# in3otd/glfer

Hardware: AMD Instinct MI355X
Metric: spectrogram frames/sec + achieved HBM GB/s, N=4096 MTM K=4 (higher is better)
Workload: dtype f32

## Files before the change

glfer_amd/csrc/odd_taper.hpp:

```cpp
#pragma once
#include "stockham16.hpp"

#ifndef GLFER_PSD_STORE_AUX
#define GLFER_PSD_STORE_AUX 0
#endif

namespace glfer {

template <int FMT, int T, int HIST = -1>
__device__ __forceinline__ void load_frame16(const SpectroParams &p, unsigned t, unsigned fl, long long fblk, float (&dst)[16]) {
  constexpr unsigned esz = FMT == GLFER_FMT_F32 ? 4 : (FMT == GLFER_FMT_S16 ? 2 : 1);
  const long long f = fblk + fl;
  const unsigned flc = f < p.nframes ? fl : (unsigned)(p.nframes - 1 - fblk);
  const long long sblk = (p.frame0 + fblk) * (long long)p.H - p.R;
  if (HIST == 1 || (HIST < 0 && p.history_mode)) {
    const __amdgpu_buffer_rsrc_t hrsrc = __builtin_amdgcn_make_buffer_rsrc(
        const_cast<char *>(reinterpret_cast<const char *>(p.stream)) + (sblk + p.R) * (long long)esz, 0, 0x7fffffff, 0x00020000);
    const int d = (int)t - p.R;
    const int lrel = (int)(flc * (unsigned)p.H) + d;
    static_for<0, 16>([&](auto mc) {
      constexpr int m = decltype(mc)::value;
      const bool ok = d >= -T * m;
      const float x = buf_sample<FMT>(hrsrc, ok ? (unsigned)(lrel + T * m) * esz : 0x80000000u, 0u);
      dst[m] = ok ? x : 0.0f;
    });
    return;
  }
  const __amdgpu_buffer_rsrc_t xrsrc = __builtin_amdgcn_make_buffer_rsrc(
      const_cast<char *>(reinterpret_cast<const char *>(p.stream)) + sblk * (long long)esz, 0, 0x7fffffff, 0x00020000);
  const unsigned lrel = flc * (unsigned)p.H + t;
  static_for<0, 16>([&](auto mc) {
    constexpr int m = decltype(mc)::value;
    dst[m] = buf_sample<FMT>(xrsrc, lrel * esz, (unsigned)(T * m) * esz);
  });
}

__device__ __forceinline__ float wave_total_f32(float v) {
  auto dpp = [](float x, auto ctrl, auto rowmask) {
    return __int_as_float(__builtin_amdgcn_update_dpp(0, __float_as_int(x), decltype(ctrl)::value, decltype(rowmask)::value, 0xf, false));
  };
  v += dpp(v, std::integral_constant<int, 0x111>{}, std::integral_constant<int, 0xf>{});
  v += dpp(v, std::integral_constant<int, 0x112>{}, std::integral_constant<int, 0xf>{});
  v += dpp(v, std::integral_constant<int, 0x114>{}, std::integral_constant<int, 0xf>{});
  v += dpp(v, std::integral_constant<int, 0x118>{}, std::integral_constant<int, 0xf>{});
  v += dpp(v, std::integral_constant<int, 0x142>{}, std::integral_constant<int, 0xa>{});
  v += dpp(v, std::integral_constant<int, 0x143>{}, std::integral_constant<int, 0xc>{});
  return __int_as_float(__builtin_amdgcn_readlane(__float_as_int(v), 63));
}

template <int FMT, int T, int KM>
__device__ __forceinline__ void load_frame16_mean(const SpectroParams &p, unsigned t, unsigned fl, long long fblk, float (&dst)[16]) {
  static_assert(T <= 64 && (KM == 16 || KM == 8 || KM == 4), "a frame within one wavefront; hop = 4, 8 or 16 registers");
  load_frame16<FMT, T, 0>(p, t, fl, fblk, dst);
  constexpr int NH = 16 / KM;
  float mu[NH];
  if (p.means) {
    const long long f = fblk + fl;
    const long long F = p.frame0 + (f < p.nframes ? f : (long long)p.nframes - 1);
#pragma unroll
    for (int q = 0; q < NH; q++) mu[q] = p.means[F - (NH - 1) + q];
  } else {
#pragma unroll
    for (int q = 0; q < NH; q++) {
      float sm = 0.0f;
#pragma unroll
      for (int m = 0; m < KM; m++) sm += dst[q * KM + m];
#pragma unroll
      for (int o = 1; o < T; o <<= 1) sm += __shfl_xor(sm, o);
      mu[q] = sm / (float)p.H;
    }
  }
#pragma unroll
  for (int m = 0; m < 16; m++) dst[m] = dst[m] - mu[m / KM];
}

constexpr int kSilent = 0x7fff;
__device__ __forceinline__ int scale_exponent(float power) {
  int ex = __builtin_amdgcn_frexp_expf(power);
  ex = ex > 120 ? 120 : (ex < -120 ? -120 : ex);
  return power == 0.0f ? kSilent : ex >> 1;
}
__device__ __forceinline__ float scale_in(int hx) { return hx == kSilent ? 0.0f : __builtin_amdgcn_ldexpf(1.0f, -hx); }
__device__ __forceinline__ float scale_out(int hx) { return hx == kSilent ? 0.0f : __builtin_amdgcn_ldexpf(1.0f, 2 * hx); }

template <int LOGN, int FPB, class SumA, class SumB>
__device__ __forceinline__ void separate_and_store(const SpectroParams &p, const float (&zr)[16], const float (&zi)[16],
                                                   v2f32 *xb, unsigned t, unsigned fl, long long fblk, int hxA, int hxB,
                                                   SumA &&sumA, SumB &&sumB) {
  using C = Plan16<LOGN>;
  constexpr int N = C::N, T = C::T, RL = C::radix(C::NPASS - 1), BL = 16 / RL;
  auto rho_of = [](int m) constexpr { return (m % BL) + BL * brev(m / BL, RL); };
  if constexpr (GLFER16_BARRIER_AFTER_READS == 0) frame_sync<T>();
  static_for<8, 16>([&](auto mc) {
    constexpr int m = decltype(mc)::value;
    constexpr int r = rho_of(m);
    xb[t + T * (m - 8)] = v2f32{zr[r], zi[r]};
  });
  frame_sync<T>();
  const unsigned ROWB = (unsigned)p.pitch * 4u;
  const long long leftA = p.nframes - fblk, leftB = p.nframes - (fblk + FPB);
  const unsigned recA = (unsigned)((leftA > FPB ? FPB : leftA) * (long long)ROWB);
  const unsigned recB = leftB > 0 ? (unsigned)((leftB > FPB ? FPB : leftB) * (long long)ROWB) : 0u;
  const __amdgpu_buffer_rsrc_t ra = __builtin_amdgcn_make_buffer_rsrc(p.psd + (size_t)fblk * (size_t)p.pitch, 0, recA, 0x00020000);
  const __amdgpu_buffer_rsrc_t rb = __builtin_amdgcn_make_buffer_rsrc(p.psd + (size_t)(fblk + (leftB > 0 ? FPB : 0)) * (size_t)p.pitch, 0, recB, 0x00020000);
  const unsigned voff = fl * ROWB + t * 4u;
  const float uA = scale_out(hxA), uB = scale_out(hxB);
  static_for<0, 8>([&](auto mc) {
    constexpr int m = decltype(mc)::value;
    constexpr int r = rho_of(m);
    const int k = (int)t + T * m;
    v2f32 b = xb[N / 2 - k];
    const float ar = zr[r], ai = zi[r];
    if constexpr (m == 0) {
      if (t == 0) b = v2f32{ar, ai};
    }
    const float er = ar + b.x, ei = ai - b.y, orr = ar - b.x, oi = ai + b.y;
    const float pa = __builtin_fmaf(er, er, ei * ei), pb = __builtin_fmaf(orr, orr, oi * oi);
    __builtin_amdgcn_raw_buffer_store_b32(__float_as_uint(__builtin_fmaf(pa, uA, sumA(mc))), ra, voff, (unsigned)(T * m) * 4u, GLFER_PSD_STORE_AUX);
    __builtin_amdgcn_raw_buffer_store_b32(__float_as_uint(__builtin_fmaf(pb, uB, sumB(mc))), rb, voff, (unsigned)(T * m) * 4u, GLFER_PSD_STORE_AUX);
  });
  if (t == 0) {
    constexpr int r = rho_of(8);
    constexpr std::integral_constant<int, 8> nyq{};
    __builtin_amdgcn_raw_buffer_store_b32(__float_as_uint(__builtin_fmaf(4.0f * zr[r] * zr[r], uA, sumA(nyq))), ra, voff, (unsigned)(N / 2) * 4u, GLFER_PSD_STORE_AUX);
    __builtin_amdgcn_raw_buffer_store_b32(__float_as_uint(__builtin_fmaf(4.0f * zi[r] * zi[r], uB, sumB(nyq))), rb, voff, (unsigned)(N / 2) * 4u, GLFER_PSD_STORE_AUX);
  }
  frame_sync<T>();
}

}
```

glfer_amd/csrc/spectro16y.hip:

```cpp
#include <hip/hip_runtime.h>
#include <stdint.h>
#include "odd_taper.hpp"

#ifndef GLFER16Y_DPP_SUM
#define GLFER16Y_DPP_SUM 1
#endif
#ifndef GLFER16Y_SKEW
#define GLFER16Y_SKEW 1
#endif
#ifndef GLFER16Y_HALF
#define GLFER16Y_HALF 1
#endif
#ifndef GLFER16Y_TW1_REGS
#define GLFER16Y_TW1_REGS 1
#endif

#ifndef GLFER_BLOCK_MARK
#define GLFER_BLOCK_MARK(k)
#endif

#ifdef GLFER_RAGGED
#define spectro16y_kernel spectro16y_ragged_kernel
#define glfer_launch_spectro16y_n12 glfer_launch_spectro16y_ragged_n12
#endif

namespace glfer {

hipError_t allow_dynamic_lds(const void *kernel, size_t bytes);

struct LaunchY {
  static constexpr int N = 4096, T = 256, PADN = N + N / 16;
  static constexpr int LDS_WORDS = 2 * PADN + 16 * 17 + 4;
};

template <int FMT, int ABL = 0, int HIST = 0, int KM = 0, int BAT = 0, int HALF = 0, int QUEUE = 0>
__global__ __launch_bounds__(256, 2) void spectro16y_kernel(SpectroParams p) {
  GLFER_BLOCK_MARK(0);
  if constexpr (KM == 0 || BAT != 0) GLFER_STREAM_SELECT(p);
  static_assert(KM == 0 || (HIST == 0 && (KM == 16 || KM == 8 || KM == 4)), "in-kernel mean removal: history from the stream");
  static_assert(HALF == 0 || (KM == 0 && GLFER16_X0_ROWS != 0 && GLFER16_BARRIER_AFTER_READS != 0), "half tables: the plain forms, row layout of exchange 0");
  static_assert(QUEUE == 0 || (KM == 0 && BAT == 0 && ABL == 0), "frame queue: the plain single-stream forms");
  constexpr int NH = KM > 0 ? 16 / KM : 1;
  __shared__ float mred[KM > 0 ? 4 * (NH + 1) : 1];
  using C = Plan16<12>;
  using L = LaunchY;
  constexpr int N = L::N, T = L::T, PADN = L::PADN, NPASS = C::NPASS;
  constexpr int TW1 = 15;
  constexpr int NT = C::NTW - TW1;
  constexpr unsigned esz = FMT == GLFER_FMT_F32 ? 4 : (FMT == GLFER_FMT_S16 ? 2 : 1);
  typedef float v4f32 __attribute__((ext_vector_type(4)));
  extern __shared__ v2f32 lds[];

  const unsigned t = threadIdx.x;
  const unsigned rc = HALF ? glfer_yhalf_residue(t) : t;
  v2f32 *xbA = lds, *xbB = lds + PADN;
  v2f32 *tw1 = lds + 2 * PADN;
  float *red = reinterpret_cast<float *>(lds + 2 * PADN + 16 * 17);

  {
    const v2f32 *tw = reinterpret_cast<const v2f32 *>(p.tw);
    const unsigned k = t >> 4, q = t & 15;
    tw1[k * 17 + q] = q ? tw[(q - 1) * T + k] : v2f32{1.0f, 0.0f};
  }
  float twr[NT], twi[NT];
  {
    const v2f32 *tw = reinterpret_cast<const v2f32 *>(p.tw) + t;
#pragma unroll
    for (int e = 0; e < NT; e++) {
      const v2f32 w = tw[(TW1 + e) * T];
      twr[e] = w.x;
      twi[e] = w.y;
    }
  }
  __syncthreads();
  const v2f32 *tw1row = tw1 + (t & 15) * 17;
  constexpr bool TW1R = GLFER16Y_TW1_REGS != 0 && HIST == 0 && KM != 4;
  v2f32 tw1reg[16];
  if constexpr (TW1R) {
#pragma unroll
    for (int q = 0; q < 16; q++) tw1reg[q] = tw1row[q];
  }

  const __amdgpu_buffer_rsrc_t trsrc = __builtin_amdgcn_make_buffer_rsrc(
      const_cast<float *>(p.taps), 0, p.npairs * 2 * N * 4, 0x00020000);
  const __amdgpu_buffer_rsrc_t vrsrc = __builtin_amdgcn_make_buffer_rsrc(
      const_cast<float *>(p.xtaps), 0, N * 4, 0x00020000);
  const unsigned toff = t * 16u;
  const int NP = p.npairs - 1;
  const long long stride = (long long)gridDim.x * 2;

  auto load_x = [&](float (&dst)[16], long long f) {
    load_frame16<FMT, T, HIST>(p, rc, 0u, f < p.nframes ? f : (long long)p.nframes - 1, dst);
  };
  v2f32 pt[16];
  auto prefetch_taps = [&](int pair) {
    const unsigned tap_p = (unsigned)pair * (N * 8u);
    static_for<0, 8>([&](auto mc) {
      constexpr int mh = decltype(mc)::value;
      const v4f32 q = __builtin_bit_cast(v4f32, __builtin_amdgcn_raw_buffer_load_b128(trsrc, toff, tap_p + (unsigned)(T * mh) * 16u, 0));
      pt[2 * mh] = v2f32{q.x, q.y};
      pt[2 * mh + 1] = v2f32{q.z, q.w};
    });
  };
  auto prefetch_last = [&] {
    static_for<0, 4>([&](auto mc) {
      constexpr int mq = decltype(mc)::value;
      const v4f32 q = __builtin_bit_cast(v4f32, __builtin_amdgcn_raw_buffer_load_b128(vrsrc, toff, (unsigned)(T * mq) * 16u, 0));
      pt[2 * mq] = v2f32{q.x, q.y};
      pt[2 * mq + 1] = v2f32{q.z, q.w};
    });
  };

  v2f32 hp[16];
  float hl[8];
  const __amdgpu_buffer_rsrc_t yrsrc = __builtin_amdgcn_make_buffer_rsrc(
      const_cast<float *>(p.ytaps), 0, HALF ? T * GLFER_YHALF_FLOATS * 4 : 0, 0x00020000);
  const unsigned yoff = t * (unsigned)(GLFER_YHALF_FLOATS * 4);
  auto load_half_last = [&] {
    static_for<0, 2>([&](auto cc) {
      constexpr int c = decltype(cc)::value;
      const v4f32 q = __builtin_bit_cast(v4f32, __builtin_amdgcn_raw_buffer_load_b128(yrsrc, yoff, 128u + c * 16u, 0));
      hl[4 * c] = q.x;
      hl[4 * c + 1] = q.y;
      hl[4 * c + 2] = q.z;
      hl[4 * c + 3] = q.w;
    });
  };
  if constexpr (HALF != 0) {
    static_for<0, 8>([&](auto cc) {
      constexpr int c = decltype(cc)::value;
      const v4f32 q = __builtin_bit_cast(v4f32, __builtin_amdgcn_raw_buffer_load_b128(yrsrc, yoff, c * 16u, 0));
      hp[2 * c] = v2f32{q.x, q.y};
      hp[2 * c + 1] = v2f32{q.z, q.w};
    });
// ... 7 lines not shown
    if constexpr (m < 8) return hp[P * 8 + m];
    else return v2f32{mirror(hp[P * 8 + 15 - m].x), -mirror(hp[P * 8 + 15 - m].y)};
  };

  const long long span = QUEUE ? 2LL * p.yq_chunk : 2;
  unsigned *qword = reinterpret_cast<unsigned *>(tw1 + 16);
  long long fA = (long long)xcd_block_index() * span;
  if (fA >= p.nframes) return;
  long long fEnd = fA + span < p.nframes ? fA + span : (long long)p.nframes, next_chunk = 0;
  bool fresh = true;
  float xA[16], xB[16];
  load_x(xA, fA);
  if (fA + 1 < p.nframes) load_x(xB, fA + 1);
  else {
#pragma unroll
    for (int m = 0; m < 16; m++) xB[m] = 0.0f;
  }
  if constexpr (HALF == 0) prefetch_taps(0);

  auto publish_hop_sums = [&] {
    static_for<0, NH + 1>([&](auto qc) {
      constexpr int q = decltype(qc)::value;
      float sm = 0.0f;
      static_for<0, KM>([&](auto mc) {
        constexpr int m = decltype(mc)::value;
        sm += q < NH ? xA[q * KM + m] : xB[(NH - 1) * KM + m];
      });
#pragma unroll
      for (int o = 1; o < 64; o <<= 1) sm += __shfl_xor(sm, o);
      if ((t & 63u) == 0) mred[(t >> 6) * (NH + 1) + q] = sm;
    });
  };
  auto subtract_hop_means = [&] {
    float mu[NH + 1];
#pragma unroll
    for (int q = 0; q <= NH; q++)
      mu[q] = ((mred[q] + mred[(NH + 1) + q]) + (mred[2 * (NH + 1) + q] + mred[3 * (NH + 1) + q])) / (float)p.H;
#pragma unroll
    for (int m = 0; m < 16; m++) {
      xA[m] = xA[m] - mu[m / (KM ? KM : 1)];
      xB[m] = xB[m] - mu[m / (KM ? KM : 1) + 1];
    }
  };
  auto subtract_table_means = [&](long long fa) {
    float mu[NH + 1];
    const long long F = p.frame0 + fa;
#pragma unroll
    for (int q = 0; q < NH; q++) mu[q] = p.means[F - (NH - 1) + q];
    mu[NH] = p.means[fa + 1 < p.nframes ? F + 1 : F];
#pragma unroll
    for (int m = 0; m < 16; m++) {
      xA[m] = xA[m] - mu[m / (KM ? KM : 1)];
      xB[m] = xB[m] - mu[m / (KM ? KM : 1) + 1];
    }
  };
  if constexpr (KM > 0) {
    if (p.means) {
      subtract_table_means(fA);
    } else {
      publish_hop_sums();
      __syncthreads();
      subtract_hop_means();
      __syncthreads();
    }
    if (fA + 1 >= p.nframes) {
#pragma unroll
      for (int m = 0; m < 16; m++) xB[m] = 0.0f;
    }
  }

  constexpr int RL = C::radix(NPASS - 1), BL = 16 / RL;
  auto rho_of = [](int m) constexpr { return (m % BL) + BL * brev(m / BL, RL); };

  GLFER_BLOCK_MARK(1);
  while (true) {
    long long nfA = fA + stride;
    bool has_next = nfA < p.nframes;
    unsigned ticket = 0;
    if constexpr (QUEUE != 0) {
      if (fresh && t == 0) ticket = __hip_atomic_fetch_add(p.yq_counter, 1u, __ATOMIC_RELAXED, __HIP_MEMORY_SCOPE_AGENT);
    }
    float psdA[8], psdB[8], nyqA, nyqB;
    int hxA, hxB;
    {
      float accA[16], accB[16];
#pragma unroll
      for (int r = 0; r < 16; r++) accA[r] = accB[r] = 0.0f;
      if constexpr (HALF != 0) {
        static_for<0, 2>([&](auto pc) {
          constexpr int P = decltype(pc)::value;
          float zrA[16], ziA[16], zrB[16], ziB[16];
          GLFER_STAMP(0);
          static_for<0, 16>([&](auto mc) {
            constexpr int m = decltype(mc)::value;
            const v2f32 w = half_pair(pc, mc);
            zrA[m] = xA[m] * w.x;
            ziA[m] = xA[m] * w.y;
            zrB[m] = xB[m] * w.x;
            ziB[m] = xB[m] * w.y;
          });
          auto dual = [&](const auto &tw1sel) {
            auto hook = [] {};
            if constexpr (GLFER16Y_SKEW != 0) stockham16_passes2s<12, NT>(zrA, ziA, xbA, zrB, ziB, xbB, t, rc, tw1sel, twr, twi, hook);
            else stockham16_passes2<12, NT>(zrA, ziA, xbA, zrB, ziB, xbB, t, rc, tw1sel, twr, twi, hook);
          };
          if constexpr (TW1R) dual(tw1reg);
          else dual(tw1row);
#pragma unroll
          for (int r = 0; r < 16; r++) {
            if constexpr (P == 0) {
              accA[r] = __builtin_fmaf(zrA[r], zrA[r], ziA[r] * ziA[r]);
              accB[r] = __builtin_fmaf(zrB[r], zrB[r], ziB[r] * ziB[r]);
            } else {
              accA[r] = __builtin_fmaf(zrA[r], zrA[r], __builtin_fmaf(ziA[r], ziA[r], accA[r]));
              accB[r] = __builtin_fmaf(zrB[r], zrB[r], __builtin_fmaf(ziB[r], ziB[r], accB[r]));
            }
          }
          GLFER_STAMP(15);
        });
        if constexpr (HALF == 2) load_half_last();
      } else
      for (int pair = 0; pair < NP; pair++) {
        float zrA[16], ziA[16], zrB[16], ziB[16];
        GLFER_STAMP(0);
#pragma unroll
        for (int m = 0; m < 16; m++) {
          zrA[m] = xA[m] * pt[m].x;
          ziA[m] = xA[m] * pt[m].y;
          zrB[m] = xB[m] * pt[m].x;
          ziB[m] = xB[m] * pt[m].y;
        }
        auto dual = [&](const auto &tw1sel) {
          auto hook = [&] {
            if (pair + 1 < NP) prefetch_taps(pair + 1);
            else prefetch_last();
          };
          if constexpr (GLFER16Y_SKEW != 0) stockham16_passes2s<12, NT>(zrA, ziA, xbA, zrB, ziB, xbB, t, tw1sel, twr, twi, hook);
          else stockham16_passes2<12, NT>(zrA, ziA, xbA, zrB, ziB, xbB, t, tw1sel, twr, twi, hook);
        };
        if constexpr (TW1R) dual(tw1reg);
        else dual(tw1row);
        if (pair == 0) {
#pragma unroll
          for (int r = 0; r < 16; r++) {
            accA[r] = __builtin_fmaf(zrA[r], zrA[r], ziA[r] * ziA[r]);
            accB[r] = __builtin_fmaf(zrB[r], zrB[r], ziB[r] * ziB[r]);
          }
        } else {
#pragma unroll
          for (int r = 0; r < 16; r++) {
            accA[r] = __builtin_fmaf(zrA[r], zrA[r], __builtin_fmaf(ziA[r], ziA[r], accA[r]));
            accB[r] = __builtin_fmaf(zrB[r], zrB[r], __builtin_fmaf(ziB[r], ziB[r], accB[r]));
          }
        }
        GLFER_STAMP(15);
      }
      float eA = 0.0f, eB = 0.0f;
#pragma unroll
      for (int r = 0; r < 16; r++) {
        eA += accA[r];
        eB += accB[r];
      }
#if GLFER16Y_DPP_SUM
      eA = wave_total_f32(eA);
      eB = wave_total_f32(eB);
#else
#pragma unroll
      for (int w = 1; w < 64; w <<= 1) {
        eA += __shfl_xor(eA, w);
        eB += __shfl_xor(eB, w);
      }
#endif
      float *foldA = reinterpret_cast<float *>(xbA), *foldB = reinterpret_cast<float *>(xbB);
      static_for<8, 16>([&](auto mc) {
        constexpr int m = decltype(mc)::value;
        foldA[t + T * (m - 8)] = accA[rho_of(m)];
        foldB[t + T * (m - 8)] = accB[rho_of(m)];
      });
      if ((t & 63) == 0) {
        red[t >> 6] = eA;
        red[4 + (t >> 6)] = eB;
      }
      if constexpr (QUEUE != 0) {
        if (fresh && t == 0) *qword = ticket - p.yq_base;
      }
      __syncthreads();
      if constexpr (QUEUE != 0) {
        if (fresh) next_chunk = ((long long)gridDim.x + (long long)(unsigned)__builtin_amdgcn_readfirstlane((int)*qword)) * span;
        nfA = fA + 2 < fEnd ? fA + 2 : next_chunk;
        has_next = nfA < p.nframes;
      }
      eA = (red[0] + red[1]) + (red[2] + red[3]);
      eB = (red[4] + red[5]) + (red[6] + red[7]);
      hxA = scale_exponent(eA);
      hxB = scale_exponent(eB);
      static_for<0, 8>([&](auto mc) {
        constexpr int m = decltype(mc)::value;
        const int k = T * m + (int)t;
        float oa = foldA[N / 2 - k], ob = foldB[N / 2 - k];
        if constexpr (m == 0) {
          if (t == 0) {
            oa = accA[rho_of(0)];
            ob = accB[rho_of(0)];
          }
        }
        psdA[m] = accA[rho_of(m)] + oa;
        psdB[m] = accB[rho_of(m)] + ob;
      });
      nyqA = 2.0f * accA[rho_of(8)];
      nyqB = 2.0f * accB[rho_of(8)];
      __syncthreads();
    }

    if constexpr (ABL == 1) {
      if (has_next) {
        if constexpr (HALF == 0) prefetch_taps(0);
        load_x(xA, nfA);
        load_x(xB, nfA + 1);
      }
      if (t == 0) p.psd[(size_t)fA * (size_t)p.pitch] = psdA[0] + psdB[0] + nyqA + nyqB + (float)(hxA + hxB);
      if (!has_next) break;
      fA = nfA;
      continue;
    }
    float zr[16], zi[16];
    GLFER_STAMP(0);
    {
      const float sA = scale_in(hxA), sB = scale_in(hxB);
      if constexpr (HALF != 0) {
        static_for<0, 16>([&](auto mc) {
          constexpr int m = decltype(mc)::value;
          float v;
          if constexpr (m < 8) v = hl[m];
          else v = mirror(hl[15 - m]);
          zr[m] = (xA[m] * v) * sA;
          zi[m] = (xB[m] * v) * sB;
        });
      } else {
#pragma unroll
        for (int m = 0; m < 16; m++) {
          const float v = (m & 1) ? pt[m / 2].y : pt[m / 2].x;
          zr[m] = (xA[m] * v) * sA;
          zi[m] = (xB[m] * v) * sB;
        }
      }
    }
    auto shared_round = [&](const auto &tw1sel) {
      auto hook = [&] {
        if (has_next) {
          if constexpr (HALF == 0) prefetch_taps(0);
          load_x(xA, nfA);
          load_x(xB, nfA + 1);
        }
      };
      if constexpr (GLFER16Y_SKEW >= 2) stockham16_passes1s<12, NT>(zr, zi, xbA, t, rc, tw1sel, twr, twi, hook);
      else stockham16_passes<12, NT>(zr, zi, xbA, t, rc, tw1sel, twr, twi, hook);
    };
    if constexpr (TW1R) shared_round(tw1reg);
    else shared_round(tw1row);
    if constexpr (KM > 0) {
      if (has_next && !p.means) publish_hop_sums();
    }
    separate_and_store<12, 1>(p, zr, zi, xbA, t, 0u, fA, hxA, hxB,
                              [&](auto mc) { if constexpr (decltype(mc)::value == 8) return nyqA; else return psdA[decltype(mc)::value]; },
                              [&](auto mc) { if constexpr (decltype(mc)::value == 8) return nyqB; else return psdB[decltype(mc)::value]; });
    GLFER_STAMP(15);
    if constexpr (KM > 0) {
      if (has_next) {
        if (p.means) subtract_table_means(nfA);
        else subtract_hop_means();
      }
    }
    if (!has_next) break;
    if constexpr (QUEUE != 0) {
      fresh = fA + 2 >= fEnd;
      if (fresh) fEnd = nfA + span < p.nframes ? nfA + span : (long long)p.nframes;
    }
    fA = nfA;
    if (fA + 1 >= p.nframes) {
#pragma unroll
      for (int m = 0; m < 16; m++) xB[m] = 0.0f;
    }
  }
  GLFER_BLOCK_MARK(2);
}

}

#ifndef GLFER_NO_LAUNCHERS
using namespace glfer;

#ifndef GLFER_RAGGED
template <int FMT>
static hipError_t launch16y_queue(const SpectroParams &p, hipStream_t st) {
  if (p.mean_inkernel || p.nbatch > 1 || p.yq_chunk < 1) return hipErrorInvalidValue;
  const unsigned grid = glfer_yq_grid(glfer_yq_chunks(p.nframes, p.yq_chunk));
  constexpr size_t shmem = (size_t)LaunchY::LDS_WORDS * 8;
#define GLFER_Y_QUEUE(HIST, HALF)                                                                                    \
  do {                                                                                                               \
    hipError_t e = allow_dynamic_lds(reinterpret_cast<const void *>(spectro16y_kernel<FMT, 0, HIST, 0, 0, HALF, 1>), shmem); \
    if (e != hipSuccess) return e;                                                                                   \
    hipLaunchKernelGGL((spectro16y_kernel<FMT, 0, HIST, 0, 0, HALF, 1>), dim3(grid), dim3(256), shmem, st, p);        \
    return hipGetLastError();                                                                                        \
  } while (0)
  if (GLFER16Y_HALF != 0 && p.ytaps && p.npairs == 3) {
    if (p.history_mode) GLFER_Y_QUEUE(1, GLFER16Y_HALF);
    else GLFER_Y_QUEUE(0, GLFER16Y_HALF);
  }
  if (p.history_mode) GLFER_Y_QUEUE(1, 0);
  else GLFER_Y_QUEUE(0, 0);
#undef GLFER_Y_QUEUE
}
#endif

template <int FMT>
static hipError_t launch16y_fmt(const SpectroParams &p, hipStream_t st) {
  const long long work = ((long long)p.nframes + 1) / 2;
  if (work == 0) return hipSuccess;
#ifdef GLFER_RAGGED
  if (p.yq_counter || !p.ragged || p.nbatch < 2) return hipErrorInvalidValue;
#else
  if (p.yq_counter) return launch16y_queue<FMT>(p, st);
#endif
  const long long resident = 256LL * 2;
  const long long cap = glfer_batch_cap(16 * resident, p.nbatch);
  unsigned grid = (unsigned)(work < cap ? work : cap);
  if (grid >= 64) grid &= ~7u;
  constexpr size_t shmem = (size_t)LaunchY::LDS_WORDS * 8;
  {
    hipError_t e = allow_dynamic_lds(reinterpret_cast<const void *>(p.history_mode ? spectro16y_kernel<FMT, 0, 1> : spectro16y_kernel<FMT, 0, 0>), shmem);
    if (e != hipSuccess) return e;
  }
  if (p.mean_inkernel) {
    if (p.history_mode) return hipErrorInvalidValue;
    const int km = p.H % 256 == 0 ? p.H / 256 : 0;
#ifdef GLFER_RAGGED
#define GLFER_Y_MEAN(K)                                                                                              \
  do {                                                                                                               \
    hipError_t e = allow_dynamic_lds(reinterpret_cast<const void *>(spectro16y_kernel<FMT, 0, 0, K, 1>), shmem);       \
    if (e != hipSuccess) return e;                                                                                   \
    hipLaunchKernelGGL((spectro16y_kernel<FMT, 0, 0, K, 1>), dim3(grid, glfer_batch_y(p)), dim3(256), shmem, st, p); \
    return hipGetLastError();                                                                                        \
  } while (0)
#else
#define GLFER_Y_MEAN(K)                                                                                              \
// ... 45 lines not shown
```

glfer_amd/csrc/stockham16.hpp:

```cpp
#pragma once
#include <hip/hip_runtime.h>
#include <stdint.h>
#include "fft_inreg.hpp"
#include "spectro_params.h"

#ifndef GLFER_STAMP
#define GLFER_STAMP(id)
#endif
#ifndef GLFER16_FOLD_TW
#define GLFER16_FOLD_TW 1
#endif
#ifndef GLFER16_BARRIER_AFTER_READS
#define GLFER16_BARRIER_AFTER_READS 1
#endif

namespace glfer {

typedef float v2f32 __attribute__((ext_vector_type(2)));

template <int LOGN>
struct Plan16 {
  static constexpr int N = 1 << LOGN;
  static constexpr int T = N / 16;
  static constexpr int NPASS = LOGN <= 8 ? 2 : (LOGN <= 12 ? 3 : 4);
  static constexpr int radix(int i) {
    if (i < 2) return 16;
    if (NPASS == 3) return N / 256;
    return i == 2 ? 16 : N / 4096;
  }
  static constexpr int ls(int i) {
    int l = 1;
    for (int j = 0; j < i; j++) l *= radix(j);
    return l;
  }
  static constexpr int tw_offset(int i) {
    int o = 0;
    for (int j = 1; j < i; j++) o += (16 / radix(j)) * (radix(j) - 1);
    return o;
  }
  static constexpr int NTW = tw_offset(NPASS);
};


template <int FMT>
__device__ __forceinline__ float cvt_sample(const void *ubase, unsigned elem_off) {
  if constexpr (FMT == GLFER_FMT_F32) {
    return *reinterpret_cast<const float *>(reinterpret_cast<const char *>(ubase) + (size_t)(elem_off * 4u));
  } else if constexpr (FMT == GLFER_FMT_S16) {
    return (float)*reinterpret_cast<const short *>(reinterpret_cast<const char *>(ubase) + (size_t)(elem_off * 2u)) / 32768.0f;
  } else {
    return ((float)*(reinterpret_cast<const unsigned char *>(ubase) + (size_t)elem_off) - 128.0f) / 128.0f;
  }
}

#ifndef GLFER_X_LOAD_AUX
#define GLFER_X_LOAD_AUX 0
#endif
template <int FMT>
__device__ __forceinline__ float buf_sample(__amdgpu_buffer_rsrc_t rsrc, unsigned voff_bytes, unsigned soff_bytes) {
  if constexpr (FMT == GLFER_FMT_F32) {
    return __uint_as_float(__builtin_amdgcn_raw_buffer_load_b32(rsrc, voff_bytes, soff_bytes, GLFER_X_LOAD_AUX));
  } else if constexpr (FMT == GLFER_FMT_S16) {
    return (float)(short)__builtin_amdgcn_raw_buffer_load_b16(rsrc, voff_bytes, soff_bytes, GLFER_X_LOAD_AUX) / 32768.0f;
  } else {
    return ((float)(unsigned char)__builtin_amdgcn_raw_buffer_load_b8(rsrc, voff_bytes, soff_bytes, GLFER_X_LOAD_AUX) - 128.0f) / 128.0f;
  }
}

__device__ __forceinline__ float limiter_value(float y) {
  const float ftmp = (float)log((double)fabsf(y));
  const float mag = (float)exp((double)ftmp * 0.1);
  return y > 0.0f ? mag : -mag;
}

__device__ __forceinline__ unsigned xcd_block_index() {
  const unsigned w = blockIdx.x, g = gridDim.x;
  return (g & 7u) ? w : (w & 7u) * (g >> 3) + (w >> 3);
}

#ifndef GLFER_ABL
#define GLFER_ABL 0
#endif
template <int T>
__device__ __forceinline__ void frame_sync() {
  if constexpr (T > 64 && !(GLFER_ABL & 1)) {
    __syncthreads();
  } else {
    __builtin_amdgcn_fence(__ATOMIC_ACQ_REL, "wavefront");
    __builtin_amdgcn_wave_barrier();
  }
// ... 111 lines not shown
      static_for<0, B>([&](auto bc) {
        constexpr int b = decltype(bc)::value;
        static_for<1, R>([&](auto qc) {
          constexpr int q = decltype(qc)::value;
          constexpr int e = C::tw_offset(i) - TW1 + b * (R - 1) + (q - 1);
          constexpr int m = b + B * q;
          const float a = zr[m], c = zi[m];
          zr[m] = __builtin_fmaf(a, twr[e], -c * twi[e]);
          zi[m] = __builtin_fmaf(a, twi[e], c * twr[e]);
        });
      });
    }
    constexpr bool kEmit = GLFER16_BARRIER_AFTER_READS != 0 && i < NPASS - 1 && B == 1;
    if constexpr (kEmit) {
      const int k = (int)t & (Ls - 1);
      const int a0 = ((int)t - k) * R + k;
      constexpr bool kRows = GLFER16_X0_ROWS != 0 && i == 0 && T >= 32;
      v2f32 *wbase = kRows ? xb + col0 : xb + a0 + (a0 >> xpad_shift(i));
      if constexpr (kFold) dit_head_tw<R, 1, 0, 16>(zr, zi, twf);
      else dit_head<R, 1, 0, 16>(zr, zi);
      dit_tail<R, 1, 0, 16>(zr, zi, [&](auto qc, auto rc) {
        constexpr int q = decltype(qc)::value, reg = decltype(rc)::value;
        if constexpr (!(GLFER_ABL & 2)) wbase[kRows ? q * (T + 2) : xpad_offset(i, q * Ls)] = v2f32{zr[reg], zi[reg]};
      });
    } else {
      static_for<0, B>([&](auto bc) {
        constexpr int b = decltype(bc)::value;
        if constexpr (kFold) dit_tw<R, B, b, 16>(zr, zi, twf);
        else dit<R, B, b, 16>(zr, zi);
      });
    }
    GLFER_STAMP(4 * i + 1);
    if constexpr (i < NPASS - 1) {
      if constexpr (GLFER16_BARRIER_AFTER_READS == 0) frame_sync<T>();
      GLFER_STAMP(4 * i + 2);
      if constexpr (!kEmit) static_for<0, B>([&](auto bc) {
        constexpr int b = decltype(bc)::value;
        const int j = (int)t + T * b;
        const int k = j & (Ls - 1);
        const int a0 = (j - k) * R + k;
        v2f32 *wbase = xb + a0 + (a0 >> xpad_shift(i));
        static_for<0, R>([&](auto qc) {
          constexpr int q = decltype(qc)::value;
          constexpr int src = b + B * brev(q, R);
          wbase[xpad_offset(i, q * Ls)] = v2f32{zr[src], zi[src]};
        });
      });
      if constexpr (i == 0) {
        after_first_write();
        __builtin_amdgcn_sched_barrier(0);
      }
      GLFER_STAMP(4 * i + 3);
      frame_sync<T>();
      GLFER_STAMP(4 * i + 4);
      if constexpr (GLFER_ABL & 4) {
      } else if constexpr (GLFER16_X0_ROWS != 0 && GLFER16_BARRIER_AFTER_READS != 0 && i == 0 && T >= 32 && B == 1) {
        v2f32 v[16];
        lds_read16_strided<T / 16>(xb + (t & 15) * (T + 2) + (t >> 4), v);
#pragma unroll
        for (int m = 0; m < 16; m++) {
          zr[m] = v[m].x;
          zi[m] = v[m].y;
        }
      } else {
        const v2f32 *rbase = xb + t + (t >> xpad_shift(i));
        constexpr int STRIDE = xpad_offset(i, T);
        if constexpr (GLFER16_X0_ROWS != 0 && T % 32 == 0 && i > 0 && 15 * STRIDE * 8 < 65536 && xpad_offset(i, 15 * T) == 15 * STRIDE) {
          v2f32 v[16];
          lds_read16_strided<STRIDE>(rbase, v);
#pragma unroll
          for (int m = 0; m < 16; m++) {
            zr[m] = v[m].x;
            zi[m] = v[m].y;
          }
        } else {
          static_for<0, 16>([&](auto mc) {
            constexpr int m = decltype(mc)::value;
            const v2f32 v = rbase[xpad_offset(i, m * T)];
            zr[m] = v.x;
            zi[m] = v.y;
          });
        }
      }
      if constexpr (GLFER16_BARRIER_AFTER_READS != 0) frame_sync<T>();
    }
  });
}

template <int LOGM, int NT, class Tw1, class Hook>
__device__ __forceinline__ void stockham16_passes2(float (&zrA)[16], float (&ziA)[16], v2f32 *xbA, float (&zrB)[16],
                                                   float (&ziB)[16], v2f32 *xbB, unsigned t, unsigned col0, const Tw1 &tw1row,
                                                   const float (&twr)[NT], const float (&twi)[NT],
                                                   Hook &&after_first_write) {
  using C = Plan16<LOGM>;
  constexpr int T = C::T, NPASS = C::NPASS, TW1 = 15;
  static_assert(GLFER16_BARRIER_AFTER_READS != 0, "stockham16_passes2 relies on the barrier-after-reads scheme");
  static_for<0, NPASS>([&](auto ic) {
    constexpr int i = decltype(ic)::value;
    constexpr int R = C::radix(i), Ls = C::ls(i), B = 16 / R;
    constexpr bool kFold = GLFER16_FOLD_TW != 0 && i > 0;
    const PassTwiddles<C, i, NT, Tw1> twf{tw1row, twr, twi};
    auto compute = [&](float (&zr)[16], float (&zi)[16], v2f32 *xb) {
      if constexpr (kFold) {
      } else if constexpr (i == 1) {
        static_for<1, 16>([&](auto qc) {
          constexpr int q = decltype(qc)::value;
          const v2f32 w = tw1row[q];
          const float a = zr[q], c = zi[q];
          zr[q] = __builtin_fmaf(a, w.x, -c * w.y);
          zi[q] = __builtin_fmaf(a, w.y, c * w.x);
        });
      } else if constexpr (i > 1) {
        static_for<0, B>([&](auto bc) {
          constexpr int b = decltype(bc)::value;
          static_for<1, R>([&](auto qc) {
            constexpr int q = decltype(qc)::value;
            constexpr int e = C::tw_offset(i) - TW1 + b * (R - 1) + (q - 1);
            constexpr int m = b + B * q;
            const float a = zr[m], c = zi[m];
            zr[m] = __builtin_fmaf(a, twr[e], -c * twi[e]);
            zi[m] = __builtin_fmaf(a, twi[e], c * twr[e]);
          });
        });
      }
      if constexpr (i < NPASS - 1) {
        static_assert(B == 1, "an exchange follows radix-16 passes only");
        const int k = (int)t & (Ls - 1);
        const int a0 = ((int)t - k) * R + k;
        constexpr bool kRows = GLFER16_X0_ROWS != 0 && i == 0 && T >= 32;
        v2f32 *wbase = kRows ? xb + col0 : xb + a0 + (a0 >> xpad_shift(i));
        if constexpr (kFold) dit_head_tw<R, 1, 0, 16>(zr, zi, twf);
        else dit_head<R, 1, 0, 16>(zr, zi);
        dit_tail<R, 1, 0, 16>(zr, zi, [&](auto qc, auto rc) {
          constexpr int q = decltype(qc)::value, reg = decltype(rc)::value;
          if constexpr (!(GLFER_ABL & 2)) wbase[kRows ? q * (T + 2) : xpad_offset(i, q * Ls)] = v2f32{zr[reg], zi[reg]};
        });
      } else {
        static_for<0, B>([&](auto bc) {
          constexpr int b = decltype(bc)::value;
          if constexpr (kFold) dit_tw<R, B, b, 16>(zr, zi, twf);
          else dit<R, B, b, 16>(zr, zi);
        });
      }
    };
    compute(zrA, ziA, xbA);
    GLFER_STAMP(4 * i + 1);
    __builtin_amdgcn_sched_barrier(0);
    compute(zrB, ziB, xbB);
    if constexpr (i < NPASS - 1) {
      if constexpr (i == 0) after_first_write();
      __builtin_amdgcn_sched_barrier(0);
      GLFER_STAMP(4 * i + 2);
      frame_sync<T>();
      GLFER_STAMP(4 * i + 3);
      if constexpr (GLFER_ABL & 4) {
      } else if constexpr (GLFER16_X0_ROWS != 0 && i == 0 && T >= 32) {
        v2f32 va[16], vb[16];
        const int roff = (int)(t & 15) * (T + 2) + (int)(t >> 4);
        lds_read16_strided<T / 16>(xbA + roff, va);
        lds_read16_strided<T / 16>(xbB + roff, vb);
#pragma unroll
        for (int m = 0; m < 16; m++) {
          zrA[m] = va[m].x;
          ziA[m] = va[m].y;
          zrB[m] = vb[m].x;
          ziB[m] = vb[m].y;
        }
// ... 126 lines not shown
        frame_sync<T>();
      }
    }
  });
}

template <int LOGM, int NT, class Tw1, class Hook>
__device__ __forceinline__ void stockham16_passes1s(float (&zr)[16], float (&zi)[16], v2f32 *xb, unsigned t, unsigned col0, const Tw1 &tw1row,
                                                    const float (&twr)[NT], const float (&twi)[NT], Hook &&after_first_write) {
  using C = Plan16<LOGM>;
  constexpr int T = C::T, NPASS = C::NPASS, TW1 = 15;
  static_assert(GLFER16_BARRIER_AFTER_READS != 0 && GLFER16_X0_ROWS != 0 && T >= 32 && T % 32 == 0 && !(GLFER_ABL & 7), "the product configuration");
  static_for<0, NPASS>([&](auto ic) {
    constexpr int i = decltype(ic)::value;
    constexpr int R = C::radix(i), Ls = C::ls(i);
    static_assert(R == 16, "radix-16 passes");
    auto tail = [&] {
      if constexpr (i < NPASS - 1) {
        const int k = (int)t & (Ls - 1);
        const int a0 = ((int)t - k) * R + k;
        constexpr bool kRows = i == 0;
        v2f32 *wbase = kRows ? xb + col0 : xb + a0 + (a0 >> xpad_shift(i));
        dit_tail<R, 1, 0, 16>(zr, zi, [&](auto qc, auto rc) {
          constexpr int q = decltype(qc)::value, reg = decltype(rc)::value;
          wbase[kRows ? q * (T + 2) : xpad_offset(i, q * Ls)] = v2f32{zr[reg], zi[reg]};
        });
      } else {
        dit_tail<R, 1, 0, 16>(zr, zi, [](auto, auto) {});
      }
    };
    if constexpr (i == 0) {
      dit_head<R, 1, 0, 16>(zr, zi);
      tail();
      after_first_write();
      __builtin_amdgcn_sched_barrier(0);
      frame_sync<T>();
    } else {
      v2f32 v[16];
      if constexpr (i == 1) {
        lds_read16_strided<T / 16>(xb + (t & 15) * (T + 2) + (t >> 4), v);
      } else {
        constexpr int STRIDE = xpad_offset(i - 1, T);
        static_assert(15 * STRIDE * 8 < 65536 && xpad_offset(i - 1, 15 * T) == 15 * STRIDE, "one stride");
        lds_read16_strided<STRIDE>(xb + t + (t >> xpad_shift(i - 1)), v);
      }
#pragma unroll
      for (int m = 0; m < 16; m++) {
        zr[m] = v[m].x;
        zi[m] = v[m].y;
      }
      if constexpr (GLFER16_FOLD_TW != 0) {
        const PassTwiddles<C, i, NT, Tw1> twf{tw1row, twr, twi};
        dit_head_tw<R, 1, 0, 16>(zr, zi, twf);
      } else {
        if constexpr (i == 1) {
          static_for<1, 16>([&](auto qc) {
            constexpr int q = decltype(qc)::value;
            const v2f32 w = tw1row[q];
            const float a = zr[q], c = zi[q];
            zr[q] = __builtin_fmaf(a, w.x, -c * w.y);
            zi[q] = __builtin_fmaf(a, w.y, c * w.x);
          });
        } else {
          static_for<1, R>([&](auto qc) {
            constexpr int q = decltype(qc)::value;
            constexpr int e = C::tw_offset(i) - TW1 + (q - 1);
            const float a = zr[q], c = zi[q];
            zr[q] = __builtin_fmaf(a, twr[e], -c * twi[e]);
            zi[q] = __builtin_fmaf(a, twi[e], c * twr[e]);
          });
        }
        dit_head<R, 1, 0, 16>(zr, zi);
      }
      frame_sync<T>();
      tail();
      if constexpr (i < NPASS - 1) {
        __builtin_amdgcn_sched_barrier(0);
        frame_sync<T>();
      }
    }
  });
}

template <int LOGM, int NT, class Tw1, class Hook>
__device__ __forceinline__ void stockham16_passes(float (&zr)[16], float (&zi)[16], v2f32 *xb, unsigned t, const Tw1 &tw1row,
                                                  const float (&twr)[NT], const float (&twi)[NT], Hook &&after_first_write) {
  stockham16_passes<LOGM, NT>(zr, zi, xb, t, t, tw1row, twr, twi, after_first_write);
}
template <int LOGM, int NT, class Tw1, class Hook>
__device__ __forceinline__ void stockham16_passes1s(float (&zr)[16], float (&zi)[16], v2f32 *xb, unsigned t, const Tw1 &tw1row,
                                                    const float (&twr)[NT], const float (&twi)[NT], Hook &&after_first_write) {
  stockham16_passes1s<LOGM, NT>(zr, zi, xb, t, t, tw1row, twr, twi, after_first_write);
}
template <int LOGM, int NT, class Tw1, class Hook>
__device__ __forceinline__ void stockham16_passes2(float (&zrA)[16], float (&ziA)[16], v2f32 *xbA, float (&zrB)[16],
                                                   float (&ziB)[16], v2f32 *xbB, unsigned t, const Tw1 &tw1row,
                                                   const float (&twr)[NT], const float (&twi)[NT], Hook &&after_first_write) {
  stockham16_passes2<LOGM, NT>(zrA, ziA, xbA, zrB, ziB, xbB, t, t, tw1row, twr, twi, after_first_write);
}
template <int LOGM, int NT, class Tw1, class Hook>
__device__ __forceinline__ void stockham16_passes2s(float (&zrA)[16], float (&ziA)[16], v2f32 *xbA, float (&zrB)[16],
                                                    float (&ziB)[16], v2f32 *xbB, unsigned t, const Tw1 &tw1row,
                                                    const float (&twr)[NT], const float (&twi)[NT], Hook &&after_first_write) {
  stockham16_passes2s<LOGM, NT>(zrA, ziA, xbA, zrB, ziB, xbB, t, t, tw1row, twr, twi, after_first_write);
}

}
```

Measured before the change: 92.44 million.

## Fold taper-sum mirror exchange into FFT final pass and ping-pong exchange buffers

Instead of writing the folded upper-half accumulator sums to LDS and exchanging them in a separate round with its own barriers, the last FFT pass now writes the mirror spectrum and both accumulator values as one 16-byte LDS entry. A single separation step then combines the spectrum and the folded sums. The FFT passes alternate between two exchange buffers, which removes the barrier after reads. The aim is to cut barriers and LDS round trips per frame pair, at the cost of keeping the accumulators live in registers through the FFT, which raises register pressure, and wider LDS entries.

```diff
diff --git a/glfer_amd/csrc/odd_taper.hpp b/glfer_amd/csrc/odd_taper.hpp
--- a/glfer_amd/csrc/odd_taper.hpp
+++ b/glfer_amd/csrc/odd_taper.hpp
@@ -96,7 +96,9 @@
     constexpr int r = rho_of(m);
     xb[t + T * (m - 8)] = v2f32{zr[r], zi[r]};
   });
+  GLFER_STAMP(12);
   frame_sync<T>();
+  GLFER_STAMP(13);
   const unsigned ROWB = (unsigned)p.pitch * 4u;
   const long long leftA = p.nframes - fblk, leftB = p.nframes - (fblk + FPB);
   const unsigned recA = (unsigned)((leftA > FPB ? FPB : leftA) * (long long)ROWB);
@@ -125,6 +127,58 @@
     __builtin_amdgcn_raw_buffer_store_b32(__float_as_uint(__builtin_fmaf(4.0f * zr[r] * zr[r], uA, sumA(nyq))), ra, voff, (unsigned)(N / 2) * 4u, GLFER_PSD_STORE_AUX);
     __builtin_amdgcn_raw_buffer_store_b32(__float_as_uint(__builtin_fmaf(4.0f * zi[r] * zi[r], uB, sumB(nyq))), rb, voff, (unsigned)(N / 2) * 4u, GLFER_PSD_STORE_AUX);
   }
+  GLFER_STAMP(14);
+  frame_sync<T>();
+}
+
+typedef float v4f32_lds __attribute__((ext_vector_type(4)));
+template <int LOGN, int M>
+__device__ __forceinline__ void mirror_entry_write(v2f32 *xb, unsigned t, float re, float im, float sa, float sb) {
+  constexpr int T = Plan16<LOGN>::T;
+  static_assert(M >= 8 && M < 16, "an upper-half bin");
+  reinterpret_cast<v4f32_lds *>(xb)[t + T * (M - 8)] = v4f32_lds{re, im, sa, sb};
+}
+template <int LOGN>
+__device__ __forceinline__ void separate_fold_and_store(const SpectroParams &p, const float (&zr)[16], const float (&zi)[16],
+                                                        const float (&accA)[16], const float (&accB)[16], v2f32 *xb, unsigned t,
+                                                        long long fblk, int hxA, int hxB) {
+  using C = Plan16<LOGN>;
+  constexpr int N = C::N, T = C::T, RL = C::radix(C::NPASS - 1), BL = 16 / RL;
+  static_assert((N / 2 + 1) * 16 <= (N + N / 16) * 8, "the mirror entries fit one exchange buffer");
+  auto rho_of = [](int m) constexpr { return (m % BL) + BL * brev(m / BL, RL); };
+  GLFER_STAMP(12);
+  frame_sync<T>();
+  GLFER_STAMP(13);
+  const unsigned ROWB = (unsigned)p.pitch * 4u;
+  const long long leftA = p.nframes - fblk, leftB = p.nframes - (fblk + 1);
+  const unsigned recA = (unsigned)((leftA > 1 ? 1 : leftA) * (long long)ROWB);
+  const unsigned recB = leftB > 0 ? ROWB : 0u;
+  const __amdgpu_buffer_rsrc_t ra = __builtin_amdgcn_make_buffer_rsrc(p.psd + (size_t)fblk * (size_t)p.pitch, 0, recA, 0x00020000);
+  const __amdgpu_buffer_rsrc_t rb = __builtin_amdgcn_make_buffer_rsrc(p.psd + (size_t)(fblk + (leftB > 0 ? 1 : 0)) * (size_t)p.pitch, 0, recB, 0x00020000);
+  const unsigned voff = t * 4u;
+  const float uA = scale_out(hxA), uB = scale_out(hxB);
+  const v4f32_lds *xe = reinterpret_cast<const v4f32_lds *>(xb);
+  static_for<0, 8>([&](auto mc) {
+    constexpr int m = decltype(mc)::value;
+    constexpr int r = rho_of(m);
+    const int k = (int)t + T * m;
+    v4f32_lds b = xe[N / 2 - k];
+    const float ar = zr[r], ai = zi[r];
+    if constexpr (m == 0) {
+      if (t == 0) b = v4f32_lds{ar, ai, accA[r], accB[r]};
+    }
+    const float sa = accA[r] + b.z, sb = accB[r] + b.w;
+    const float er = ar + b.x, ei = ai - b.y, orr = ar - b.x, oi = ai + b.y;
+    const float pa = __builtin_fmaf(er, er, ei * ei), pb = __builtin_fmaf(orr, orr, oi * oi);
+    __builtin_amdgcn_raw_buffer_store_b32(__float_as_uint(__builtin_fmaf(pa, uA, sa)), ra, voff, (unsigned)(T * m) * 4u, GLFER_PSD_STORE_AUX);
+    __builtin_amdgcn_raw_buffer_store_b32(__float_as_uint(__builtin_fmaf(pb, uB, sb)), rb, voff, (unsigned)(T * m) * 4u, GLFER_PSD_STORE_AUX);
+  });
+  if (t == 0) {
+    constexpr int r = rho_of(8);
+    __builtin_amdgcn_raw_buffer_store_b32(__float_as_uint(__builtin_fmaf(4.0f * zr[r] * zr[r], uA, 2.0f * accA[r])), ra, voff, (unsigned)(N / 2) * 4u, GLFER_PSD_STORE_AUX);
+    __builtin_amdgcn_raw_buffer_store_b32(__float_as_uint(__builtin_fmaf(4.0f * zi[r] * zi[r], uB, 2.0f * accB[r])), rb, voff, (unsigned)(N / 2) * 4u, GLFER_PSD_STORE_AUX);
+  }
+  GLFER_STAMP(14);
   frame_sync<T>();
 }
 
diff --git a/glfer_amd/csrc/spectro16y.hip b/glfer_amd/csrc/spectro16y.hip
--- a/glfer_amd/csrc/spectro16y.hip
+++ b/glfer_amd/csrc/spectro16y.hip
@@ -22,6 +22,13 @@
 #ifdef GLFER_RAGGED
 #define spectro16y_kernel spectro16y_ragged_kernel
 #define glfer_launch_spectro16y_n12 glfer_launch_spectro16y_ragged_n12
+#endif
+#ifndef GLFER16Y_ONE_MIRROR_PASS
+#ifdef GLFER_RAGGED
+#define GLFER16Y_ONE_MIRROR_PASS 0
+#else
+#define GLFER16Y_ONE_MIRROR_PASS 1
+#endif
 #endif
 
 namespace glfer {
@@ -40,6 +47,8 @@
   static_assert(KM == 0 || (HIST == 0 && (KM == 16 || KM == 8 || KM == 4)), "in-kernel mean removal: history from the stream");
   static_assert(HALF == 0 || (KM == 0 && GLFER16_X0_ROWS != 0 && GLFER16_BARRIER_AFTER_READS != 0), "half tables: the plain forms, row layout of exchange 0");
   static_assert(QUEUE == 0 || (KM == 0 && BAT == 0 && ABL == 0), "frame queue: the plain single-stream forms");
+  constexpr bool SEG = HALF != 0 && GLFER16Y_ONE_MIRROR_PASS != 0;
+  static_assert(!SEG || ABL == 0, "the ablation reads the folded sums in front of the shared round");
   constexpr int NH = KM > 0 ? 16 / KM : 1;
   __shared__ float mred[KM > 0 ? 4 * (NH + 1) : 1];
   using C = Plan16<12>;
@@ -49,7 +58,7 @@
   constexpr int NT = C::NTW - TW1;
   constexpr unsigned esz = FMT == GLFER_FMT_F32 ? 4 : (FMT == GLFER_FMT_S16 ? 2 : 1);
   typedef float v4f32 __attribute__((ext_vector_type(4)));
-  extern __shared__ v2f32 lds[];
+  extern __shared__ __attribute__((aligned(16))) v2f32 lds[];
 
   const unsigned t = threadIdx.x;
   const unsigned rc = HALF ? glfer_yhalf_residue(t) : t;
@@ -223,8 +232,8 @@
     }
     float psdA[8], psdB[8], nyqA, nyqB;
     int hxA, hxB;
+    float accA[16], accB[16];
     {
-      float accA[16], accB[16];
 #pragma unroll
       for (int r = 0; r < 16; r++) accA[r] = accB[r] = 0.0f;
       if constexpr (HALF != 0) {
@@ -312,8 +321,9 @@
         eB += __shfl_xor(eB, w);
       }
 #endif
-      float *foldA = reinterpret_cast<float *>(xbA), *foldB = reinterpret_cast<float *>(xbB);
-      static_for<8, 16>([&](auto mc) {
+      GLFER_SEG_STAMP(0);
+      [[maybe_unused]] float *foldA = reinterpret_cast<float *>(xbA), *foldB = reinterpret_cast<float *>(xbB);
+      if constexpr (!SEG) static_for<8, 16>([&](auto mc) {
         constexpr int m = decltype(mc)::value;
         foldA[t + T * (m - 8)] = accA[rho_of(m)];
         foldB[t + T * (m - 8)] = accB[rho_of(m)];
@@ -325,7 +335,9 @@
       if constexpr (QUEUE != 0) {
         if (fresh && t == 0) *qword = ticket - p.yq_base;
       }
+      GLFER_SEG_STAMP(1);
       __syncthreads();
+      GLFER_SEG_STAMP(2);
       if constexpr (QUEUE != 0) {
         if (fresh) next_chunk = ((long long)gridDim.x + (long long)(unsigned)__builtin_amdgcn_readfirstlane((int)*qword)) * span;
         nfA = fA + 2 < fEnd ? fA + 2 : next_chunk;
@@ -335,6 +347,7 @@
       eB = (red[4] + red[5]) + (red[6] + red[7]);
       hxA = scale_exponent(eA);
       hxB = scale_exponent(eB);
+      if constexpr (!SEG) {
       static_for<0, 8>([&](auto mc) {
         constexpr int m = decltype(mc)::value;
         const int k = T * m + (int)t;
@@ -350,7 +363,9 @@
       });
       nyqA = 2.0f * accA[rho_of(8)];
       nyqB = 2.0f * accB[rho_of(8)];
+      GLFER_SEG_STAMP(3);
       __syncthreads();
+      }
     }
 
     if constexpr (ABL == 1) {
@@ -394,6 +409,12 @@
           load_x(xB, nfA + 1);
         }
       };
+      if constexpr (SEG) {
+        stockham16_passes_pp<12, NT>(zr, zi, xbA, xbB, t, rc, tw1sel, twr, twi, hook, [&](auto qc, auto regc) {
+          constexpr int q = decltype(qc)::value, reg = decltype(regc)::value;
+          if constexpr (q >= 8) mirror_entry_write<12, q>(xbA, t, zr[reg], zi[reg], accA[reg], accB[reg]);
+        });
+      } else
       if constexpr (GLFER16Y_SKEW >= 2) stockham16_passes1s<12, NT>(zr, zi, xbA, t, rc, tw1sel, twr, twi, hook);
       else stockham16_passes<12, NT>(zr, zi, xbA, t, rc, tw1sel, twr, twi, hook);
     };
@@ -402,6 +423,8 @@
     if constexpr (KM > 0) {
       if (has_next && !p.means) publish_hop_sums();
     }
+    if constexpr (SEG) separate_fold_and_store<12>(p, zr, zi, accA, accB, xbA, t, fA, hxA, hxB);
+    else
     separate_and_store<12, 1>(p, zr, zi, xbA, t, 0u, fA, hxA, hxB,
                               [&](auto mc) { if constexpr (decltype(mc)::value == 8) return nyqA; else return psdA[decltype(mc)::value]; },
                               [&](auto mc) { if constexpr (decltype(mc)::value == 8) return nyqB; else return psdB[decltype(mc)::value]; });
diff --git a/glfer_amd/csrc/stockham16.hpp b/glfer_amd/csrc/stockham16.hpp
--- a/glfer_amd/csrc/stockham16.hpp
+++ b/glfer_amd/csrc/stockham16.hpp
@@ -6,6 +6,9 @@
 
 #ifndef GLFER_STAMP
 #define GLFER_STAMP(id)
+#endif
+#ifndef GLFER_SEG_STAMP
+#define GLFER_SEG_STAMP(id)
 #endif
 #ifndef GLFER16_FOLD_TW
 #define GLFER16_FOLD_TW 1
@@ -283,7 +286,9 @@
           });
         }
       }
+      GLFER_SEG_STAMP(4 + i);
       if constexpr (GLFER16_BARRIER_AFTER_READS != 0) frame_sync<T>();
+      GLFER_SEG_STAMP(6 + i);
     }
   });
 }
@@ -576,6 +581,60 @@
   });
 }
 
+template <int LOGM, int NT, class Tw1, class Hook, class Emit>
+__device__ __forceinline__ void stockham16_passes_pp(float (&zr)[16], float (&zi)[16], v2f32 *xb0, v2f32 *xb1, unsigned t, unsigned col0,
+                                                     const Tw1 &tw1row, const float (&twr)[NT], const float (&twi)[NT],
+                                                     Hook &&after_first_write, Emit &&last_emit) {
+  using C = Plan16<LOGM>;
+  constexpr int T = C::T, NPASS = C::NPASS;
+  static_assert(NPASS == 3 && GLFER16_FOLD_TW != 0 && GLFER16_BARRIER_AFTER_READS != 0 && GLFER16_X0_ROWS != 0 && T >= 32 && T % 32 == 0 && !(GLFER_ABL & 7),
+                "the product configuration, three passes");
+  static_for<0, NPASS>([&](auto ic) {
+    constexpr int i = decltype(ic)::value;
+    constexpr int R = C::radix(i), Ls = C::ls(i);
+    static_assert(R == 16, "radix-16 passes");
+    const PassTwiddles<C, i, NT, Tw1> twf{tw1row, twr, twi};
+    if constexpr (i == 0) dit_head<R, 1, 0, 16>(zr, zi);
+    else dit_head_tw<R, 1, 0, 16>(zr, zi, twf);
+    if constexpr (i == NPASS - 1) {
+      dit_tail<R, 1, 0, 16>(zr, zi, last_emit);
+      GLFER_STAMP(4 * i + 1);
+    } else {
+      v2f32 *xb = i == 0 ? xb0 : xb1;
+      const int k = (int)t & (Ls - 1);
+      const int a0 = ((int)t - k) * R + k;
+      constexpr bool kRows = i == 0;
+      v2f32 *wbase = kRows ? xb + col0 : xb + a0 + (a0 >> xpad_shift(i));
+      dit_tail<R, 1, 0, 16>(zr, zi, [&](auto qc, auto rc) {
+        constexpr int q = decltype(qc)::value, reg = decltype(rc)::value;
+        wbase[kRows ? q * (T + 2) : xpad_offset(i, q * Ls)] = v2f32{zr[reg], zi[reg]};
+      });
+      GLFER_STAMP(4 * i + 1);
+      if constexpr (i == 0) {
+        after_first_write();
+        __builtin_amdgcn_sched_barrier(0);
+      }
+      GLFER_STAMP(4 * i + 3);
+      frame_sync<T>();
+      GLFER_STAMP(4 * i + 4);
+      v2f32 v[16];
+      if constexpr (i == 0) {
+        lds_read16_strided<T / 16>(xb + (t & 15) * (T + 2) + (t >> 4), v);
+      } else {
+        constexpr int STRIDE = xpad_offset(i, T);
+        static_assert(15 * STRIDE * 8 < 65536 && xpad_offset(i, 15 * T) == 15 * STRIDE, "one stride");
+        lds_read16_strided<STRIDE>(xb + t + (t >> xpad_shift(i)), v);
+      }
+#pragma unroll
+      for (int m = 0; m < 16; m++) {
+        zr[m] = v[m].x;
+        zi[m] = v[m].y;
+      }
+      GLFER_SEG_STAMP(4 + i);
+    }
+  });
+}
+
 template <int LOGM, int NT, class Tw1, class Hook>
 __device__ __forceinline__ void stockham16_passes(float (&zr)[16], float (&zi)[16], v2f32 *xb, unsigned t, const Tw1 &tw1row,
                                                   const float (&twr)[NT], const float (&twi)[NT], Hook &&after_first_write) {
```

Measured after the change: 94.09 million (median of 6 runs). 1.02x the previous value.
